# mitmul/chainer-faster-rcnn

Measured on AMD Instinct MI355X. Metric: images/sec VGG16 Faster R-CNN 600x1000, higher is better.
Workload: dtype f32; 1 GPU; VGG16 inference, 1xMI355X per image, batch 1, 300 proposals post-NMS, fp32 (BASELINE.json configs[1]); 1 image per GPU per step; image=1x3x600x1000, global_batch=1, launch=hipGraph replay, parallelism=dp1 (images sharded, no collective), n_rois_last_step=300

## Files before the change

chainer-faster-rcnn_amd/_lib.py:

```python
import ctypes
import os

HERE = os.path.dirname(os.path.abspath(__file__))
LIB_PATH = os.path.join(HERE, "libfrcnn_hip.so")

_P = ctypes.c_void_p
_I = ctypes.c_int
_D = ctypes.c_double
_F = ctypes.c_float
_S = ctypes.c_size_t

SIGNATURES = {
    "frcnn_abi_version": (_I, []),
    "frcnn_device_count": (_I, []),
    "frcnn_set_tuning": (_I, [ctypes.c_char_p, ctypes.c_char_p]),
    "frcnn_get_tuning": (_I, [ctypes.c_char_p, ctypes.c_char_p, _I]),
    "frcnn_reset_tuning": (_I, []),
    "frcnn_nms_workspace_bytes": (_S, [_I]),
    "frcnn_nms": (_I, [_P, _I, _D, _I, _P, _P, _P, _S, _P]),
    "frcnn_nms_batched_workspace_bytes": (_S, [_I, _I]),
    "frcnn_nms_batched": (_I, [_P, _I, _I, _D, _I, _P, _P, _P, _S, _P]),
    "frcnn_proposals_workspace_bytes": (_S, [_I, _I, _I, _I]),
    "frcnn_proposals": (_I, [_P, _P, _I, _I, _I, _P, _I, _I, _I, _F, _I, _I, _D, _P, _P, _P, _P, _P, _S, _P]),
    "frcnn_roi_pool_workspace_bytes": (_S, [_I, _I, _I]),
    "frcnn_chw_to_hwc": (_I, [_P, _I, _I, _I, _P, _P]),
    "frcnn_roi_pool_fwd_hwc": (_I, [_P, _I, _I, _I, _P, _I, _I, _I, _I, _F, _P, _P, _P]),
    "frcnn_roi_pool_fwd_chw": (_I, [_P, _I, _I, _I, _P, _I, _I, _I, _I, _F, _P, _P, _P, _S, _P]),
    "frcnn_roi_pool_fwd_chw_bf16": (_I, [_P, _I, _I, _I, _P, _I, _I, _I, _I, _F, _P, _P]),
    "frcnn_roi_pool_fwd_blk_bf16": (_I, [_P, _I, _I, _I, _P, _I, _I, _I, _I, _F, _P, _I, _P]),
    "frcnn_roi_pool_fwd_chw_f32s": (_I, [_P, _I, _I, _I, _P, _I, _I, _I, _I, _F, _P, _P]),
    "frcnn_roi_pool_fwd": (_I, [_P, _I, _I, _I, _P, _I, _I, _I, _F, _P, _P, _P, _S, _P]),
    "frcnn_roi_pool_bwd": (_I, [_P, _P, _I, _I, _I, _I, _I, _I, _P, _P]),
    "frcnn_roi_pool_bwd_ordered": (_I, [_P, _P, _I, _I, _I, _I, _I, _I, _P, _P]),
    "frcnn_pack_conv3x3_w": (_I, [_P, _I, _I, _P, _P]),
    "frcnn_conv3x3_workspace_bytes": (_S, [_I, _I, _I, _I]),
    "frcnn_conv3x3_workspace_init": (_I, [_P, _S, _P]),
    "frcnn_conv3x3_f32": (_I, [_P, _P, _P, _P, _I, _I, _I, _I, _I, _P, _S, _P]),
    "frcnn_conv3x3_f32_cfg": (_I, [_P, _P, _P, _P, _I, _I, _I, _I, _I, _I, _P, _S, _P]),
    "frcnn_wino_pack_w": (_I, [_P, _I, _I, _I, _P, _P]),
    "frcnn_conv_wino_workspace_bytes": (_S, [_I, _I, _I, _I]),
    "frcnn_conv3x3_wino_f32": (_I, [_P, _P, _P, _P, _I, _I, _I, _I, _I, _P, _S, _P]),
    "frcnn_maxpool2x2_f32": (_I, [_P, _P, _I, _I, _I, _P]),
    "frcnn_rpn_heads_padded_channels": (_I, [_I]),
    "frcnn_rpn_heads_pack": (_I, [_P, _P, _P, _P, _I, _I, _P, _P, _P]),
    "frcnn_rpn_heads_f32": (_I, [_P, _I, _I, _I, _I, _P, _P, _P, _P, _P]),
    "frcnn_linear_workspace_bytes": (_S, [_I, _I, _I]),
    "frcnn_linear_f32": (_I, [_P, _P, _P, _P, _I, _I, _I, _I, _P, _S, _P]),
    "frcnn_head_decode": (_I, [_P, _P, _P, _I, _I, _I, _I, _P, _P, _P]),
    "frcnn_head_decode_stacked": (_I, [_P, _P, _I, _I, _I, _I, _I, _I, _P, _P, _P]),
    "frcnn_preprocess_u8": (_I, [_P, _I, _I, _I, _P, _D, _I, _I, _P, _P]),
    "frcnn_class_dets": (_I, [_P, _P, _I, _I, _P, _P]),
    "frcnn_bbox_transform_inv": (_I, [_P, _P, _I, _I, _P, _P]),
    "frcnn_clip_boxes": (_I, [_P, _I, _I, _I, _P]),
    "frcnn_softmax_rows": (_I, [_P, _I, _I, _P, _P]),
    "frcnn_conv_f32_ex": (_I, [_P, _P, _P, _P, _P, _I, _I, _I, _I, _I, _I, _P, _S, _P]),
    "frcnn_f32s_pack_conv_w": (_I, [_P, _I, _I, _P, _P]),
    "frcnn_f32s_from_nchw_f32": (_I, [_P, _I, _I, _I, _P, _P]),
    "frcnn_f32s_to_nchw_f32": (_I, [_P, _I, _I, _I, _P, _P]),
    "frcnn_conv3x3_f32s": (_I, [_P, _P, _P, _P, _I, _I, _I, _I, _I, _I, _P]),
    "frcnn_conv1_f32s": (_I, [_P, _P, _P, _P, _I, _I, _I, _I, _I, _P]),
    "frcnn_conv1_bf16": (_I, [_P, _P, _P, _P, _I, _I, _I, _I, _I, _P]),
    "frcnn_conv1_f32": (_I, [_P, _P, _P, _P, _I, _I, _I, _I, _I, _P]),
    "frcnn_f32s_pack_from_packed": (_I, [_P, _I, _I, _I, _P, _P]),
    "frcnn_f32s_pack_many": (_I, [_P, _I, _P]),
    "frcnn_conv_wgrad_f32s": (_I, [_P, _P, _P, _I, _I, _I, _I, _P, _S, _P]),
    "frcnn_conv1_f32s_train": (_I, [_P, _P, _P, _P, _P, _I, _I, _I, _I, _I, _P]),
    "frcnn_conv3x3_f32s_train": (_I, [_P, _P, _P, _P, _P, _P, _I, _I, _I, _I, _I, _P, _S, _P]),
    "frcnn_bf16_pack_many": (_I, [_P, _I, _P]),
    "frcnn_conv1_bf16_train": (_I, [_P, _P, _P, _P, _P, _I, _I, _I, _I, _I, _P]),
    "frcnn_conv3x3_bf16_train": (_I, [_P, _P, _P, _P, _P, _P, _I, _I, _I, _I, _I, _P, _S, _P]),
    "frcnn_conv_wgrad_bf16_workspace_bytes": (_S, [_I, _I, _I, _I]),
    "frcnn_conv_wgrad_bf16": (_I, [_P, _P, _P, _I, _I, _I, _I, _P, _S, _P]),
    "frcnn_f16_pack_many": (_I, [_P, _I, _P]),
    "frcnn_conv1_f16_train": (_I, [_P, _P, _P, _P, _P, _I, _I, _I, _I, _I, _P]),
# ... 157 lines not shown
```

chainer-faster-rcnn_amd/csrc/conv_wino.hip:

```cpp
#include "frcnn_common.h"
#include <frcnn_buffer.h>
#include <frcnn_intrin.h>

typedef float f32x16 __attribute__((ext_vector_type(16)));

namespace {

constexpr int kWinoPitch = 40;
constexpr int kWinoLead = 3;

template <int CB, int TB, int CK, int BPC, bool SOFF>
__global__ void __launch_bounds__(256, BPC)
conv_wino_f32_kernel(const float *__restrict__ x, const float *__restrict__ u, const float *__restrict__ bias, float *__restrict__ y,
                     int Cin, int Cout, int H, int W, int mode, int xtiles, int ytiles, int nchunks, int piece_chunks) {
    constexpr int NT = 256;
    constexpr int BCO = 32 * CB;
    constexpr int HR = 4 * TB + 2;
    constexpr int WV = CK * 4 * BCO;
    constexpr int WIT = WV / NT;
    constexpr int HG = CK * HR * 10;
    constexpr int HIT4 = (HG + NT - 1) / NT;
    constexpr int HVP = (HG + 63) / 64 * 256;
    constexpr int WBUF = WV * 4;
    constexpr int ZF = 4 * 2 * TB * CB * 16 * 64;
    constexpr int MAINF = 2 * WBUF + 2 * HVP;
    constexpr int SMEM = MAINF > ZF ? MAINF : ZF;
    static_assert(WV % NT == 0, "U slab must split into whole per-thread float4s");
    static_assert(CK % 2 == 0 && CK * HR * 3 <= NT, "chunk shape");
    static_assert(SMEM * 4 <= 160 * 1024, "LDS");
    __shared__ __attribute__((aligned(16))) float smem[SMEM];

    const int tid = threadIdx.x, lane = tid & 63;
    const int wave = __builtin_amdgcn_readfirstlane(tid >> 6);
    const int l31 = lane & 31, khalf = lane >> 5;
    const int HW = H * W;
    const int npx = xtiles * ytiles, ntiles = npx * (Cout / BCO);
    int g = blockIdx.x;
    {
        const int G = gridDim.x, xcd = g & 7, q = G >> 3, r = G & 7;
        g = xcd * q + (xcd < r ? xcd : r) + (g >> 3);
    }
    const int piece = g / ntiles, tile = g % ntiles;
    const int pxt = tile % npx, cot = tile / npx;
    const int tx = pxt % xtiles, ty = pxt / xtiles;
    const int x0 = tx * 32, y0 = ty * 4 * TB, co0 = cot * BCO;
    const int c_begin = piece * piece_chunks;
    const int c_end = nchunks < c_begin + piece_chunks ? nchunks : c_begin + piece_chunks;
    const int K4 = Cin * 4;

    const frcnn_buf_t xbuf = frcnn_make_buf(x, (uint32_t)((size_t)Cin * HW * sizeof(float)));
    const frcnn_buf_t ubuf = frcnn_make_buf(u, (uint32_t)((size_t)K4 * Cout * 4 * sizeof(float)));
    const uint32_t u_chunk_bytes = (uint32_t)(CK * 4 * Cout * 4) * 4u, x_chunk_bytes = (uint32_t)(CK * HW) * 4u;

    uint32_t woff[WIT], hoff[HIT4];
#pragma unroll
    for (int q = 0; q < WIT; ++q) {
        const int v = tid + q * NT;
        const int row = v / BCO, c4 = v % BCO;
        woff[q] = (uint32_t)(row * Cout * 4 + (co0 + c4) * 4) * 4u;
    }
#pragma unroll
    for (int q = 0; q < HIT4; ++q) {
        const int e4 = tid + q * NT;
        const int c = e4 / (HR * 10), rem = e4 % (HR * 10);
        const int hr = rem / 10, g4 = rem % 10;
        const int gy = y0 - 1 + hr, gx = x0 - 4 + 4 * g4;
        const bool inside = e4 < HG && gy >= 0 && gy < H && gx >= 0 && gx < W;
        hoff[q] = inside ? (uint32_t)(c * HW + gy * W + gx) * 4u : kBufOob;
    }
    auto w_lds = [&](int buf) { return smem + buf * WBUF; };
    auto in_lds = [&](int buf) { return smem + 2 * WBUF + buf * HVP; };
    const int fix_lo = W - x0 + 4, fix_hi = (fix_lo + 3) & ~3;
    const bool edge_fix = (W & 3) != 0 && fix_lo > 0 && fix_lo < kWinoPitch;
    auto edge_zero = [&](int buf) {
        const int row = tid / 3, i = fix_lo + tid % 3;
        if (row < CK * HR && i < fix_hi) in_lds(buf)[row * kWinoPitch + i] = 0.0f;
        frcnn_barrier_nofence();
    };
    auto issue = [&](int chunk, int buf) {
        if constexpr (SOFF) {
            const uint32_t wb = (uint32_t)chunk * u_chunk_bytes, xb = (uint32_t)chunk * x_chunk_bytes;
#pragma unroll
            for (int q = 0; q < WIT; ++q) frcnn_buf_load_lds_b128(ubuf, w_lds(buf) + (q * NT + wave * 64) * 4, woff[q], wb);
#pragma unroll
            for (int q = 0; q < HIT4; ++q)
                if ((q + 1) * NT * 4 <= HVP || (wave * 64 + q * NT) * 4 < HVP)
                    frcnn_buf_load_lds_b128(xbuf, in_lds(buf) + (q * NT + wave * 64) * 4, hoff[q], xb);
        } else {
            const long long wrem = (long long)(K4 - chunk * CK * 4) * Cout * 4, xrem = (long long)(Cin - chunk * CK) * HW;
            const frcnn_buf_t ub_c = frcnn_make_buf(u + (size_t)chunk * CK * 4 * Cout * 4, (uint32_t)((wrem > 0 ? wrem : 0) * sizeof(float)));
            const frcnn_buf_t xb_c = frcnn_make_buf(x + (size_t)chunk * CK * HW, (uint32_t)((xrem > 0 ? xrem : 0) * sizeof(float)));
#pragma unroll
            for (int q = 0; q < WIT; ++q) frcnn_buf_load_lds_b128(ub_c, w_lds(buf) + (q * NT + wave * 64) * 4, woff[q], 0);
#pragma unroll
            for (int q = 0; q < HIT4; ++q)
                if ((q + 1) * NT * 4 <= HVP || (wave * 64 + q * NT) * 4 < HVP)
                    frcnn_buf_load_lds_b128(xb_c, in_lds(buf) + (q * NT + wave * 64) * 4, hoff[q], 0);
        }
    };

    f32x16 acc[TB][4][CB];
#pragma unroll
    for (int t = 0; t < TB; ++t)
#pragma unroll
        for (int k = 0; k < 4; ++k)
#pragma unroll
            for (int c = 0; c < CB; ++c)
#pragma unroll
                for (int r = 0; r < 16; ++r) acc[t][k][c][r] = 0.0f;

    const int ra = wave == 0 ? 0 : (wave == 2 ? 2 : 1);
    const int rb = wave == 0 ? 2 : (wave == 1 ? 2 : (wave == 2 ? 1 : 3));
    const float sb = wave == 1 ? 1.0f : -1.0f;
    const int tr = l31 >> 4, tc = l31 & 15;

    issue(c_begin, 0);
    frcnn_wait_vmcnt<0>();
    frcnn_barrier_nofence();
    if (edge_fix) edge_zero(0);
    int cur = 0;
    for (int chunk = c_begin; chunk < c_end; ++chunk) {
        const bool more = chunk + 1 < c_end;
        if (more) issue(chunk + 1, cur ^ 1);
        constexpr int NSTEP = CK / 2;
        const float *b_base = in_lds(cur) + (khalf * HR + 2 * tr) * kWinoPitch + kWinoLead + 2 * tc;
        const float *ba = b_base + ra * kWinoPitch, *bb = b_base + rb * kWinoPitch;
        const float4 *a_base = reinterpret_cast<const float4 *>(w_lds(cur)) + (khalf * 4 + wave) * BCO + l31;
        auto frag = [&](int s, float4 *a, float (*da)[4], float (*db)[4]) {
#pragma unroll
            for (int c = 0; c < CB; ++c) a[c] = a_base[2 * s * 4 * BCO + 32 * c];
#pragma unroll
            for (int t = 0; t < TB; ++t)
#pragma unroll
                for (int j = 0; j < 4; ++j) {
                    da[t][j] = ba[(2 * s * HR + 4 * t) * kWinoPitch + j];
                    db[t][j] = bb[(2 * s * HR + 4 * t) * kWinoPitch + j];
                }
        };
        float4 a[2][CB];
        float da[2][TB][4], db[2][TB][4];
        frag(0, a[0], da[0], db[0]);
#pragma unroll
        for (int s = 0; s < NSTEP; ++s) {
            if (s + 1 < NSTEP) frag(s + 1, a[(s + 1) & 1], da[(s + 1) & 1], db[(s + 1) & 1]);
            __builtin_amdgcn_sched_barrier(0);
#pragma unroll
            for (int t = 0; t < TB; ++t) {
                float tt[4];
#pragma unroll
                for (int j = 0; j < 4; ++j) tt[j] = fmaf(sb, db[s & 1][t][j], da[s & 1][t][j]);
                const float v[4] = {tt[0] - tt[2], tt[1] + tt[2], tt[2] - tt[1], tt[1] - tt[3]};
#pragma unroll
                for (int c = 0; c < CB; ++c) {
                    const float4 av = a[s & 1][c];
                    acc[t][0][c] = __builtin_amdgcn_mfma_f32_32x32x2f32(av.x, v[0], acc[t][0][c], 0, 0, 0);
                    acc[t][1][c] = __builtin_amdgcn_mfma_f32_32x32x2f32(av.y, v[1], acc[t][1][c], 0, 0, 0);
                    acc[t][2][c] = __builtin_amdgcn_mfma_f32_32x32x2f32(av.z, v[2], acc[t][2][c], 0, 0, 0);
                    acc[t][3][c] = __builtin_amdgcn_mfma_f32_32x32x2f32(av.w, v[3], acc[t][3][c], 0, 0, 0);
                }
            }
        }
        frcnn_wait_vmcnt<0>();
        frcnn_barrier_nofence();
        if (edge_fix && more) edge_zero(cur ^ 1);
        cur ^= 1;
    }

    float4 *z4 = reinterpret_cast<float4 *>(smem);
#pragma unroll
    for (int t = 0; t < TB; ++t)
#pragma unroll
        for (int c = 0; c < CB; ++c)
#pragma unroll
            for (int r4 = 0; r4 < 4; ++r4) {
                float z0[4], z1[4];
#pragma unroll
                for (int e = 0; e < 4; ++e) {
                    const int r = 4 * r4 + e;
                    z0[e] = (acc[t][0][c][r] + acc[t][1][c][r]) + acc[t][2][c][r];
                    z1[e] = (acc[t][1][c][r] - acc[t][2][c][r]) - acc[t][3][c][r];
                }
                z4[(((wave * 2 + 0) * TB * CB + t * CB + c) * 4 + r4) * 64 + lane] = make_float4(z0[0], z0[1], z0[2], z0[3]);
                z4[(((wave * 2 + 1) * TB * CB + t * CB + c) * 4 + r4) * 64 + lane] = make_float4(z1[0], z1[1], z1[2], z1[3]);
            }
    __syncthreads();
    const bool relu = (mode & 1) != 0, pool = (mode & 2) != 0, partial = (mode & 4) != 0;
    const int OH = (H + 1) / 2, OW = (W + 1) / 2;
#pragma unroll
    for (int t = 0; t < TB; ++t) {
        const int oy = y0 + 4 * t + 2 * tr, ox = x0 + 2 * tc;
        const bool in0 = oy < H && ox < W, has_r = ox + 1 < W, has_d = oy + 1 < H;
#pragma unroll
        for (int c = 0; c < CB; ++c) {
            float4 zz[4][2];
#pragma unroll
            for (int r = 0; r < 4; ++r)
#pragma unroll
                for (int q = 0; q < 2; ++q) zz[r][q] = z4[(((r * 2 + q) * TB * CB + t * CB + c) * 4 + wave) * 64 + lane];
            const int cob = co0 + 32 * c + 8 * wave + 4 * khalf;
            const float4 bq = partial ? make_float4(0.f, 0.f, 0.f, 0.f) : *reinterpret_cast<const float4 *>(&bias[cob]);
#pragma unroll
            for (int e = 0; e < 4; ++e) {
                auto comp = [&](const float4 &v) { return e == 0 ? v.x : (e == 1 ? v.y : (e == 2 ? v.z : v.w)); };
                float yv[2][2];
#pragma unroll
                for (int q = 0; q < 2; ++q) {
                    yv[0][q] = (comp(zz[0][q]) + comp(zz[1][q])) + comp(zz[2][q]);
                    yv[1][q] = (comp(zz[1][q]) - comp(zz[2][q])) - comp(zz[3][q]);
                }
                const float b = comp(bq);
                const int co = cob + e;
                if (!in0) continue;
                if (pool) {
                    float m = yv[0][0];
                    if (has_r) m = fmaxf(m, yv[0][1]);
                    if (has_d) m = fmaxf(m, yv[1][0]);
                    if (has_r && has_d) m = fmaxf(m, yv[1][1]);
                    y[(size_t)co * OH * OW + (size_t)(oy >> 1) * OW + (ox >> 1)] = fmaxf(m + b, 0.0f);
                } else {
                    float *yo = y + (partial ? (size_t)piece * Cout * HW : 0) + (size_t)co * HW + (size_t)oy * W + ox;
#pragma unroll
                    for (int p = 0; p < 2; ++p)
#pragma unroll
                        for (int q = 0; q < 2; ++q) {
                            if ((p && !has_d) || (q && !has_r)) continue;
                            float v = yv[p][q] + b;
                            if (relu) v = fmaxf(v, 0.0f);
                            yo[p * W + q] = v;
                        }
                }
            }
        }
    }
}

__global__ void __launch_bounds__(256)
wino_combine_kernel(const float *__restrict__ ws, const float *__restrict__ bias, float *__restrict__ y, int P, int C, int H, int W, int mode) {
    const size_t HW = (size_t)H * W, slab = (size_t)C * HW;
    const bool relu = (mode & 1) != 0, pool = (mode & 2) != 0;
    const int OH = pool ? (H + 1) / 2 : H, OW = pool ? (W + 1) / 2 : W;
    const size_t total = (size_t)C * OH * OW;
    for (size_t i = (size_t)blockIdx.x * blockDim.x + threadIdx.x; i < total; i += (size_t)gridDim.x * blockDim.x) {
        const int ow = (int)(i % OW), oh = (int)((i / OW) % OH), c = (int)(i / ((size_t)OW * OH));
        auto sum = [&](int yy, int xx) {
            const float *p = ws + (size_t)c * HW + (size_t)yy * W + xx;
            float s = p[0];
            for (int k = 1; k < P; ++k) s += p[(size_t)k * slab];
            return s;
        };
        if (pool) {
            const int yy = 2 * oh, xx = 2 * ow;
            float m = sum(yy, xx);
            if (xx + 1 < W) m = fmaxf(m, sum(yy, xx + 1));
            if (yy + 1 < H) m = fmaxf(m, sum(yy + 1, xx));
            if (xx + 1 < W && yy + 1 < H) m = fmaxf(m, sum(yy + 1, xx + 1));
            y[i] = fmaxf(m + bias[c], 0.0f);
        } else {
            float v = sum(oh, ow) + bias[c];
            y[i] = relu ? fmaxf(v, 0.0f) : v;
        }
    }
}

__global__ void __launch_bounds__(256)
wino_pack_w_kernel(const float *__restrict__ w, int Cout, int Cin, int packed, float *__restrict__ u) {
// ... 44 lines not shown
        hipLaunchKernelGGL(HIP_KERNEL_NAME(conv_wino_f32_kernel<CB, TB, CK, BPC, true>), dim3(G), dim3(256), 0, stream, x, u, bias, out, Cin, Cout, H, W,
                           kmode, p.xtiles, p.ytiles, p.nchunks, p.piece_chunks);
    else
        hipLaunchKernelGGL(HIP_KERNEL_NAME(conv_wino_f32_kernel<CB, TB, CK, BPC, false>), dim3(G), dim3(256), 0, stream, x, u, bias, out, Cin, Cout, H, W,
                           kmode, p.xtiles, p.ytiles, p.nchunks, p.piece_chunks);
    if (split) {
        const size_t total = (size_t)Cout * ((mode & 2) ? (size_t)((H + 1) / 2) * ((W + 1) / 2) : (size_t)H * W);
        const int blocks = (int)((total + 255) / 256 < 8192 ? (total + 255) / 256 : 8192);
        hipLaunchKernelGGL(wino_combine_kernel, dim3(blocks), dim3(256), 0, stream, (const float *)workspace, bias, y, p.pieces, Cout, H, W, mode);
    }
    return frcnn_launch_status();
}

static int pick_wino_config(int Cin, int Cout, int H, int W) {
    const int forced = frcnn_tune_int("FRCNN_CONV_WINO_CFG", 0);
    if (forced >= 1 && forced <= 2) return forced;
    (void)Cin; (void)Cout; (void)H; (void)W;
    return 1;
}

static int pick_wino_pieces(int cfg, int Cin, int Cout, int H, int W) {
    const int forced = frcnn_tune_int("FRCNN_CONV_WINO_SPLIT", 0);
    if (forced > 0) return forced;
    const int CK = cfg == 1 ? 8 : 4, BPC = 2;
    const long ntiles = (long)frcnn_cdiv(W, 32) * frcnn_cdiv(H, 4) * (Cout / 64);
    const long slots = (long)frcnn_cu_count() * BPC;
    const int nchunks = frcnn_cdiv(Cin, CK);
    if (ntiles >= 2 * slots) return 1;
    int pieces = (int)((2 * slots + ntiles - 1) / ntiles);
    const int maxp = nchunks / 4 > 1 ? nchunks / 4 : 1;
    return pieces < maxp ? pieces : maxp;
}

}

extern "C" {

int frcnn_wino_pack_w(const float *w, int Cout, int Cin, int packed, float *u, void *stream) {
    if (!w || !u || Cout < 1 || Cin < 1 || (packed != 0 && packed != 1)) return FRCNN_ERR_INVALID;
    hipLaunchKernelGGL(wino_pack_w_kernel, dim3(frcnn_cdiv(Cout * Cin, 256)), dim3(256), 0, (hipStream_t)stream, w, Cout, Cin, packed, u);
    return frcnn_launch_status();
}

size_t frcnn_conv_wino_workspace_bytes(int Cin, int Cout, int H, int W) {
    if (Cin < 1 || Cout < 1 || H < 1 || W < 1) return 0;
    size_t best = 256;
    for (int cfg = 1; cfg <= 2; ++cfg) {
        const int CK = cfg == 1 ? 8 : 4;
        int pieces = pick_wino_pieces(cfg, Cin, Cout, H, W);
        const int nchunks = frcnn_cdiv(Cin, CK);
        if (pieces > nchunks) pieces = nchunks;
        const int pc = frcnn_cdiv(nchunks, pieces > 0 ? pieces : 1);
        pieces = frcnn_cdiv(nchunks, pc);
        const size_t b = pieces > 1 ? frcnn_align256((size_t)pieces * Cout * H * W * sizeof(float)) : 256;
        if (b > best) best = b;
    }
    return best;
}

int frcnn_conv3x3_wino_f32(const float *x, const float *u, const float *bias, float *y, int Cin, int Cout, int H, int W, int act,
                           void *workspace, size_t workspace_bytes, void *stream_) {
    hipStream_t stream = (hipStream_t)stream_;
    if (!x || !u || !bias || !y || Cin < 1 || Cout < 1 || H < 1 || W < 1 || (Cout % 64) != 0) return FRCNN_ERR_INVALID;
    if (act != 0 && act != 1 && act != 4) return FRCNN_ERR_INVALID;
    if ((size_t)Cin * H * W * 4 >= (1ull << 31) || (size_t)Cin * 16 * Cout * 4 >= (1ull << 31)) return FRCNN_ERR_INVALID;
    const int mode = act == 4 ? 3 : act;
    const int cfg = pick_wino_config(Cin, Cout, H, W);
    const int pieces = pick_wino_pieces(cfg, Cin, Cout, H, W);
    switch (cfg) {
        case 2: return launch_wino<2, 1, 4, 2>(x, u, bias, y, Cin, Cout, H, W, mode, pieces, workspace, workspace_bytes, stream);
        default: return launch_wino<2, 1, 8, 2>(x, u, bias, y, Cin, Cout, H, W, mode, pieces, workspace, workspace_bytes, stream);
    }
}

}
```

chainer-faster-rcnn_amd/runtime.py:

```python
import ctypes

import numpy as np

from . import _lib
from . import tuning as _tuning

_NP = {"f32": np.float32, "i32": np.int32, "u8": np.uint8, "f64": np.float64, "i64": np.int64, "i16": np.int16}


class TorchDeviceMemory(object):

    def __init__(self, device="cuda:0"):
        import torch
        if not torch.cuda.is_available():
            raise _lib.FrcnnError("no HIP device visible to PyTorch: the MI355X path cannot run (no CPU fallback)")
        self.torch = torch
        self.device = torch.device(device)
        self._dt = {"f32": torch.float32, "i32": torch.int32, "u8": torch.uint8, "f64": torch.float64,
                    "i64": torch.int64, "i16": torch.int16}

    def empty(self, shape, dtype="f32"):
        return self.torch.empty(shape, dtype=self._dt[dtype], device=self.device)

    def zeros(self, shape, dtype="f32"):
# ... 403 lines not shown
                   "frcnn_bbox_transform_inv")
        return pred

    def clip_boxes_(self, boxes, im_h, im_w):
        m, L = self.mem, self.lib
        n = int(np.prod(boxes.shape)) // 4
        _lib.check(L.frcnn_clip_boxes(m.ptr(boxes), n, int(im_h), int(im_w), m.stream()), "frcnn_clip_boxes")
        return boxes

    def softmax_rows(self, scores):
        m, L = self.mem, self.lib
        R, n = int(scores.shape[0]), int(scores.shape[1])
        out = m.empty((R, n), "f32")
        _lib.check(L.frcnn_softmax_rows(m.ptr(scores), R, n, m.ptr(out), m.stream()), "frcnn_softmax_rows")
        return out


    def pack_wino_w(self, w, out=None):
        m, L = self.mem, self.lib
        packed = w.ndim == 2
        co, ci = (int(w.shape[1]), int(w.shape[0]) // 9) if packed else (int(w.shape[0]), int(w.shape[1]))
        u = out if out is not None else m.empty((ci * 16, co), "f32")
        assert tuple(u.shape) == (ci * 16, co)
        _lib.check(L.frcnn_wino_pack_w(m.ptr(w), co, ci, int(packed), m.ptr(u), m.stream()), "frcnn_wino_pack_w")
        return u

    def conv3x3_wino(self, x, u, bias, act=1, out=None):
        m, L = self.mem, self.lib
        ci, H, W = [int(v) for v in x.shape[-3:]]
        co = int(u.shape[1])
        assert int(u.shape[0]) == ci * 16
        oh, ow = ((H + 1) // 2, (W + 1) // 2) if act == 4 else (H, W)
        y = out if out is not None else m.empty((1, co, oh, ow), "f32")
        ws = self.workspace("conv_wino", L.frcnn_conv_wino_workspace_bytes(ci, co, H, W))
        _lib.check(L.frcnn_conv3x3_wino_f32(m.ptr(x), m.ptr(u), m.ptr(bias), m.ptr(y), ci, co, H, W, int(act), m.ptr(ws), ws.shape[0],
                                            m.stream()), "frcnn_conv3x3_wino_f32")
        return y

    def conv_ex(self, x, w_packed, bias, ksize=3, act=1, mask=None, out=None):
        m, L = self.mem, self.lib
        ci, H, W = [int(v) for v in x.shape[-3:]]
        co = int(w_packed.shape[1])
        assert int(w_packed.shape[0]) == ci * ksize * ksize
        oh, ow = ((H + 1) // 2, (W + 1) // 2) if act == 4 else (H, W)
        y = out if out is not None else m.empty((1, co, oh, ow), "f32")
        ws = self._conv_workspace(ci, co, H, W)
        _lib.check(L.frcnn_conv_f32_ex(m.ptr(x), m.ptr(w_packed), m.ptr(bias), m.ptr(mask), m.ptr(y), ci, co, H, W, int(ksize),
                                       int(act), m.ptr(ws), ws.shape[0], m.stream()), "frcnn_conv_f32_ex")
        return y

    def f32s_pack_conv_w(self, w):
        m, L = self.mem, self.lib
        co, ci = int(w.shape[0]), int(w.shape[1])
        wp = m.empty((3, self.bf16_pad(ci) // 16, 9, self.bf16_pad(co), 16), "i16")
        _lib.check(L.frcnn_f32s_pack_conv_w(m.ptr(w), co, ci, m.ptr(wp), m.stream()), "frcnn_f32s_pack_conv_w")
        return wp

    def f32s_from_nchw(self, x):
        m, L = self.mem, self.lib
        C, H, W = [int(v) for v in x.shape[-3:]]
        y = m.empty((3, self.bf16_pad(C) // 16, H, W, 16), "i16")
        _lib.check(L.frcnn_f32s_from_nchw_f32(m.ptr(x), C, H, W, m.ptr(y), m.stream()), "frcnn_f32s_from_nchw_f32")
        return y

    def f32s_to_nchw(self, x, C):
        m, L = self.mem, self.lib
# ... 571 lines not shown
```

include/frcnn_hip.h:

```cpp
#ifndef FRCNN_HIP_H
#define FRCNN_HIP_H
#include <stddef.h>
#include <stdint.h>

#ifdef __cplusplus
extern "C" {
#endif

#define FRCNN_OK 0
#define FRCNN_ERR_INVALID (-1)
#define FRCNN_ERR_UNSUPPORTED (-2)

int frcnn_abi_version(void);
int frcnn_device_count(void);

int frcnn_set_tuning(const char *key, const char *value);
int frcnn_get_tuning(const char *key, char *value_out, int capacity);
int frcnn_reset_tuning(void);

size_t frcnn_nms_workspace_bytes(int n);
int frcnn_nms(const float *dets, int n, double thresh, int max_out, int32_t *keep, int32_t *n_keep,
              void *workspace, size_t workspace_bytes, void *stream);

size_t frcnn_nms_batched_workspace_bytes(int groups, int n);
// ... 13 lines not shown
size_t frcnn_roi_pool_workspace_bytes(int C, int H, int W);
int frcnn_chw_to_hwc(const float *x, int C, int H, int W, float *xt, void *stream);
int frcnn_roi_pool_fwd_hwc(const float *xt, int C, int H, int W, const float *rois, int R, int roi_cols,
                           int outh, int outw, float spatial_scale, float *y, int32_t *argmax, void *stream);
int frcnn_roi_pool_fwd_chw(const float *x, int C, int H, int W, const float *rois, int R, int roi_cols,
                           int outh, int outw, float spatial_scale, float *y, int32_t *argmax, void *workspace,
                           size_t workspace_bytes, void *stream);
int frcnn_roi_pool_fwd_chw_f32s(const float *x, int C, int H, int W, const float *rois, int R, int roi_cols, int outh, int outw,
                                float spatial_scale, uint16_t *y_parts, void *stream);
int frcnn_roi_pool_fwd_chw_bf16(const float *x, int C, int H, int W, const float *rois, int R, int roi_cols, int outh,
                                int outw, float spatial_scale, uint16_t *y, void *stream);
int frcnn_roi_pool_fwd_blk_bf16(const uint16_t *x_blk, int C, int H, int W, const float *rois, int R, int roi_cols, int outh,
                                int outw, float spatial_scale, void *y, int out_bf16, void *stream);
int frcnn_roi_pool_fwd(const float *x, int C, int H, int W, const float *rois, int R, int outh, int outw,
                       float spatial_scale, float *y, int32_t *argmax, void *workspace,
                       size_t workspace_bytes, void *stream);
int frcnn_roi_pool_bwd(const float *dy, const int32_t *argmax, int R, int C, int H, int W, int outh,
                       int outw, float *dx, void *stream);

int frcnn_pack_conv3x3_w(const float *w, int Cout, int Cin, float *w_packed, void *stream);
size_t frcnn_conv3x3_workspace_bytes(int Cin, int Cout, int H, int W);
int frcnn_conv3x3_workspace_init(void *workspace, size_t workspace_bytes, void *stream);
int frcnn_conv3x3_f32(const float *x, const float *w_packed, const float *bias, float *y, int Cin,
                      int Cout, int H, int W, int relu, void *workspace, size_t workspace_bytes,
                      void *stream);
int frcnn_conv3x3_f32_cfg(const float *x, const float *w_packed, const float *bias, float *y, int Cin,
                          int Cout, int H, int W, int relu, int cfg, void *workspace,
                          size_t workspace_bytes, void *stream);
int frcnn_maxpool2x2_f32(const float *x, float *y, int C, int H, int W, void *stream);
int frcnn_wino_pack_w(const float *w, int Cout, int Cin, int packed, float *u, void *stream);
size_t frcnn_conv_wino_workspace_bytes(int Cin, int Cout, int H, int W);
int frcnn_conv3x3_wino_f32(const float *x, const float *u, const float *bias, float *y, int Cin, int Cout, int H, int W, int act,
                           void *workspace, size_t workspace_bytes, void *stream);

int frcnn_rpn_heads_padded_channels(int A);
int frcnn_rpn_heads_pack(const float *w_cls, const float *b_cls, const float *w_bbox, const float *b_bbox,
                         int Cmid, int A, float *w_packed, float *b_packed, void *stream);
int frcnn_rpn_heads_f32(const float *h, int Cmid, int H, int W, int A, const float *w_packed,
                        const float *b_packed, float *raw, float *cls_prob, void *stream);

size_t frcnn_linear_workspace_bytes(int M, int N, int K);
int frcnn_linear_f32(const float *x, const float *w, const float *bias, float *y, int M, int N, int K,
                     int relu, void *workspace, size_t workspace_bytes, void *stream);

int frcnn_head_decode(const float *boxes, const float *deltas, const float *cls_score, int R, int ncls,
                      int im_h, int im_w, float *pred_boxes, float *cls_prob, void *stream);
int frcnn_head_decode_stacked(const float *boxes, const float *out, int ld, int dcol, int R, int ncls, int im_h, int im_w,
                              float *pred_boxes, float *cls_prob, void *stream);
int frcnn_class_dets(const float *cls_prob, const float *pred_boxes, int R, int ncls, float *dets, void *stream);
int frcnn_preprocess_u8(const uint8_t *img, int H, int W, int C, const double *means_host, double im_scale, int OH, int OW,
                        float *out, void *stream);
int frcnn_bbox_transform_inv(const float *boxes, const float *deltas, int R, int ncls, float *pred_boxes,
                             void *stream);
int frcnn_clip_boxes(float *boxes, int n_boxes, int im_h, int im_w, void *stream);
int frcnn_softmax_rows(const float *scores, int R, int n, float *probs, void *stream);

int frcnn_conv_f32_ex(const float *x, const float *w_packed, const float *bias, const float *mask, float *y, int Cin,
                      int Cout, int H, int W, int ksize, int act, void *workspace, size_t workspace_bytes,
                      void *stream);

int frcnn_f32s_pack_conv_w(const float *w, int Cout, int Cin, uint16_t *w_packed, void *stream);
int frcnn_f32s_from_nchw_f32(const float *x, int C, int H, int W, uint16_t *y, void *stream);
int frcnn_f32s_to_nchw_f32(const uint16_t *x, int C, int H, int W, float *y, void *stream);
int frcnn_conv3x3_f32s(const uint16_t *x, const uint16_t *w_packed, const float *bias, void *y, int Cin, int Cout, int H,
                       int W, int relu, int out_mode, void *stream);
int frcnn_conv1_f32s(const float *x, const float *w, const float *bias, uint16_t *y, int Cin, int Cout, int H, int W, int relu,
// ... 205 lines not shown
```

Baseline: 380.1 img/s.

## Add stream-K Winograd conv kernel with in-kernel split-K fixup via tile counters

Result: faster. 393.1 img/s, median of 6 (+3.4%).

```diff
diff --git a/chainer-faster-rcnn_amd/_lib.py b/chainer-faster-rcnn_amd/_lib.py
--- a/chainer-faster-rcnn_amd/_lib.py
+++ b/chainer-faster-rcnn_amd/_lib.py
@@ -40,6 +40,9 @@
     "frcnn_wino_pack_w": (_I, [_P, _I, _I, _I, _P, _P]),
     "frcnn_conv_wino_workspace_bytes": (_S, [_I, _I, _I, _I]),
     "frcnn_conv3x3_wino_f32": (_I, [_P, _P, _P, _P, _I, _I, _I, _I, _I, _P, _S, _P]),
+    "frcnn_conv_wino_sk_workspace_bytes": (_S, [_I, _I, _I, _I]),
+    "frcnn_conv_wino_sk_workspace_init": (_I, [_P, _S, _P]),
+    "frcnn_conv3x3_wino_sk_f32": (_I, [_P, _P, _P, _P, _I, _I, _I, _I, _I, _P, _S, _P]),
     "frcnn_maxpool2x2_f32": (_I, [_P, _P, _I, _I, _I, _P]),
     "frcnn_rpn_heads_padded_channels": (_I, [_I]),
     "frcnn_rpn_heads_pack": (_I, [_P, _P, _P, _P, _I, _I, _P, _P, _P]),
diff --git a/chainer-faster-rcnn_amd/csrc/conv_wino.hip b/chainer-faster-rcnn_amd/csrc/conv_wino.hip
--- a/chainer-faster-rcnn_amd/csrc/conv_wino.hip
+++ b/chainer-faster-rcnn_amd/csrc/conv_wino.hip
@@ -1,4 +1,5 @@
 #include "frcnn_common.h"
+#include <frcnn_sync.h>
 #include <frcnn_buffer.h>
 #include <frcnn_intrin.h>
 
@@ -9,43 +10,34 @@
 constexpr int kWinoPitch = 40;
 constexpr int kWinoLead = 3;
 
-template <int CB, int TB, int CK, int BPC, bool SOFF>
-__global__ void __launch_bounds__(256, BPC)
-conv_wino_f32_kernel(const float *__restrict__ x, const float *__restrict__ u, const float *__restrict__ bias, float *__restrict__ y,
-                     int Cin, int Cout, int H, int W, int mode, int xtiles, int ytiles, int nchunks, int piece_chunks) {
-    constexpr int NT = 256;
-    constexpr int BCO = 32 * CB;
-    constexpr int HR = 4 * TB + 2;
-    constexpr int WV = CK * 4 * BCO;
-    constexpr int WIT = WV / NT;
-    constexpr int HG = CK * HR * 10;
-    constexpr int HIT4 = (HG + NT - 1) / NT;
-    constexpr int HVP = (HG + 63) / 64 * 256;
-    constexpr int WBUF = WV * 4;
-    constexpr int ZF = 4 * 2 * TB * CB * 16 * 64;
-    constexpr int MAINF = 2 * WBUF + 2 * HVP;
-    constexpr int SMEM = MAINF > ZF ? MAINF : ZF;
+template <int CB, int TB, int CK>
+struct WinoGeom {
+    static constexpr int NT = 256;
+    static constexpr int BCO = 32 * CB;
+    static constexpr int HR = 4 * TB + 2;
+    static constexpr int WV = CK * 4 * BCO;
+    static constexpr int WIT = WV / NT;
+    static constexpr int HG = CK * HR * 10;
+    static constexpr int HIT4 = (HG + NT - 1) / NT;
+    static constexpr int HVP = (HG + 63) / 64 * 256;
+    static constexpr int WBUF = WV * 4;
+    static constexpr int ZF = 4 * 2 * TB * CB * 16 * 64;
+    static constexpr int MAINF = 2 * WBUF + 2 * HVP;
+    static constexpr int SMEM = MAINF > ZF ? MAINF : ZF;
     static_assert(WV % NT == 0, "U slab must split into whole per-thread float4s");
     static_assert(CK % 2 == 0 && CK * HR * 3 <= NT, "chunk shape");
     static_assert(SMEM * 4 <= 160 * 1024, "LDS");
-    __shared__ __attribute__((aligned(16))) float smem[SMEM];
-
+};
+
+template <int CB, int TB, int CK, bool SOFF>
+__device__ __forceinline__ void wino_tile_loop(float *smem, const float *__restrict__ x, const float *__restrict__ u, int Cin, int Cout, int H, int W,
+                                               int x0, int y0, int co0, int c_begin, int c_end, f32x16 (&acc)[TB][4][CB]) {
+    using Geo = WinoGeom<CB, TB, CK>;
+    constexpr int NT = Geo::NT, BCO = Geo::BCO, HR = Geo::HR, WIT = Geo::WIT, HG = Geo::HG, HIT4 = Geo::HIT4, HVP = Geo::HVP, WBUF = Geo::WBUF;
     const int tid = threadIdx.x, lane = tid & 63;
     const int wave = __builtin_amdgcn_readfirstlane(tid >> 6);
     const int l31 = lane & 31, khalf = lane >> 5;
     const int HW = H * W;
-    const int npx = xtiles * ytiles, ntiles = npx * (Cout / BCO);
-    int g = blockIdx.x;
-    {
-        const int G = gridDim.x, xcd = g & 7, q = G >> 3, r = G & 7;
-        g = xcd * q + (xcd < r ? xcd : r) + (g >> 3);
-    }
-    const int piece = g / ntiles, tile = g % ntiles;
-    const int pxt = tile % npx, cot = tile / npx;
-    const int tx = pxt % xtiles, ty = pxt / xtiles;
-    const int x0 = tx * 32, y0 = ty * 4 * TB, co0 = cot * BCO;
-    const int c_begin = piece * piece_chunks;
-    const int c_end = nchunks < c_begin + piece_chunks ? nchunks : c_begin + piece_chunks;
     const int K4 = Cin * 4;
 
     const frcnn_buf_t xbuf = frcnn_make_buf(x, (uint32_t)((size_t)Cin * HW * sizeof(float)));
@@ -99,7 +91,6 @@
         }
     };
 
-    f32x16 acc[TB][4][CB];
 #pragma unroll
     for (int t = 0; t < TB; ++t)
 #pragma unroll
@@ -166,6 +157,12 @@
         cur ^= 1;
     }
 
+}
+
+template <int CB, int TB>
+__device__ __forceinline__ void wino_z_exchange(float *smem, const f32x16 (&acc)[TB][4][CB]) {
+    const int lane = threadIdx.x & 63;
+    const int wave = __builtin_amdgcn_readfirstlane(threadIdx.x >> 6);
     float4 *z4 = reinterpret_cast<float4 *>(smem);
 #pragma unroll
     for (int t = 0; t < TB; ++t)
@@ -184,53 +181,226 @@
                 z4[(((wave * 2 + 1) * TB * CB + t * CB + c) * 4 + r4) * 64 + lane] = make_float4(z1[0], z1[1], z1[2], z1[3]);
             }
     __syncthreads();
+}
+
+template <int CB, int TB>
+__device__ __forceinline__ void wino_y_of_z(const float *smem, int t, int c, float (&yv)[4][2][2]) {
+    const int lane = threadIdx.x & 63;
+    const int wave = __builtin_amdgcn_readfirstlane(threadIdx.x >> 6);
+    const float4 *z4 = reinterpret_cast<const float4 *>(smem);
+    float4 zz[4][2];
+#pragma unroll
+    for (int r = 0; r < 4; ++r)
+#pragma unroll
+        for (int q = 0; q < 2; ++q) zz[r][q] = z4[(((r * 2 + q) * TB * CB + t * CB + c) * 4 + wave) * 64 + lane];
+#pragma unroll
+    for (int e = 0; e < 4; ++e) {
+        auto comp = [&](const float4 &v) { return e == 0 ? v.x : (e == 1 ? v.y : (e == 2 ? v.z : v.w)); };
+#pragma unroll
+        for (int q = 0; q < 2; ++q) {
+            yv[e][0][q] = (comp(zz[0][q]) + comp(zz[1][q])) + comp(zz[2][q]);
+            yv[e][1][q] = (comp(zz[1][q]) - comp(zz[2][q])) - comp(zz[3][q]);
+        }
+    }
+}
+
+__device__ __forceinline__ void wino_emit(float *__restrict__ y, const float (&yv)[2][2], float b, int co, int oy, int ox, int H, int W, bool relu,
+                                          bool pool, bool has_r, bool has_d, size_t base) {
+    if (pool) {
+        const int OH = (H + 1) / 2, OW = (W + 1) / 2;
+        float m = yv[0][0];
+        if (has_r) m = fmaxf(m, yv[0][1]);
+        if (has_d) m = fmaxf(m, yv[1][0]);
+        if (has_r && has_d) m = fmaxf(m, yv[1][1]);
+        y[(size_t)co * OH * OW + (size_t)(oy >> 1) * OW + (ox >> 1)] = fmaxf(m + b, 0.0f);
+    } else {
+        float *yo = y + base + (size_t)co * H * W + (size_t)oy * W + ox;
+#pragma unroll
+        for (int p = 0; p < 2; ++p)
+#pragma unroll
+            for (int q = 0; q < 2; ++q) {
+                if ((p && !has_d) || (q && !has_r)) continue;
+                float v = yv[p][q] + b;
+                if (relu) v = fmaxf(v, 0.0f);
+                yo[p * W + q] = v;
+            }
+    }
+}
+
+template <int CB, int TB, int CK, int BPC, bool SOFF>
+__global__ void __launch_bounds__(256, BPC)
+conv_wino_f32_kernel(const float *__restrict__ x, const float *__restrict__ u, const float *__restrict__ bias, float *__restrict__ y,
+                     int Cin, int Cout, int H, int W, int mode, int xtiles, int ytiles, int nchunks, int piece_chunks) {
+    using Geo = WinoGeom<CB, TB, CK>;
+    constexpr int BCO = Geo::BCO;
+    __shared__ __attribute__((aligned(16))) float smem[Geo::SMEM];
+
+    const int tid = threadIdx.x, lane = tid & 63;
+    const int wave = __builtin_amdgcn_readfirstlane(tid >> 6);
+    const int l31 = lane & 31, khalf = lane >> 5;
+    const int HW = H * W;
+    const int npx = xtiles * ytiles, ntiles = npx * (Cout / BCO);
+    int g = blockIdx.x;
+    {
+        const int G = gridDim.x, xcd = g & 7, q = G >> 3, r = G & 7;
+        g = xcd * q + (xcd < r ? xcd : r) + (g >> 3);
+    }
+    const int piece = g / ntiles, tile = g % ntiles;
+    const int pxt = tile % npx, cot = tile / npx;
+    const int tx = pxt % xtiles, ty = pxt / xtiles;
+    const int x0 = tx * 32, y0 = ty * 4 * TB, co0 = cot * BCO;
+    const int c_begin = piece * piece_chunks;
+    const int c_end = nchunks < c_begin + piece_chunks ? nchunks : c_begin + piece_chunks;
+
+    f32x16 acc[TB][4][CB];
+    wino_tile_loop<CB, TB, CK, SOFF>(smem, x, u, Cin, Cout, H, W, x0, y0, co0, c_begin, c_end, acc);
+    wino_z_exchange<CB, TB>(smem, acc);
     const bool relu = (mode & 1) != 0, pool = (mode & 2) != 0, partial = (mode & 4) != 0;
-    const int OH = (H + 1) / 2, OW = (W + 1) / 2;
+    const int tr = l31 >> 4, tc = l31 & 15;
 #pragma unroll
     for (int t = 0; t < TB; ++t) {
         const int oy = y0 + 4 * t + 2 * tr, ox = x0 + 2 * tc;
         const bool in0 = oy < H && ox < W, has_r = ox + 1 < W, has_d = oy + 1 < H;
 #pragma unroll
         for (int c = 0; c < CB; ++c) {
-            float4 zz[4][2];
-#pragma unroll
-            for (int r = 0; r < 4; ++r)
-#pragma unroll
-                for (int q = 0; q < 2; ++q) zz[r][q] = z4[(((r * 2 + q) * TB * CB + t * CB + c) * 4 + wave) * 64 + lane];
+            float yv[4][2][2];
+            wino_y_of_z<CB, TB>(smem, t, c, yv);
             const int cob = co0 + 32 * c + 8 * wave + 4 * khalf;
             const float4 bq = partial ? make_float4(0.f, 0.f, 0.f, 0.f) : *reinterpret_cast<const float4 *>(&bias[cob]);
 #pragma unroll
             for (int e = 0; e < 4; ++e) {
-                auto comp = [&](const float4 &v) { return e == 0 ? v.x : (e == 1 ? v.y : (e == 2 ? v.z : v.w)); };
-                float yv[2][2];
-#pragma unroll
-                for (int q = 0; q < 2; ++q) {
-                    yv[0][q] = (comp(zz[0][q]) + comp(zz[1][q])) + comp(zz[2][q]);
-                    yv[1][q] = (comp(zz[1][q]) - comp(zz[2][q])) - comp(zz[3][q]);
+                const float b = e == 0 ? bq.x : (e == 1 ? bq.y : (e == 2 ? bq.z : bq.w));
+                if (!in0) continue;
+                wino_emit(y, yv[e], b, cob + e, oy, ox, H, W, relu, pool, has_r, has_d, partial ? (size_t)piece * Cout * HW : 0);
+            }
+        }
+    }
+}
+
+template <bool SOFF>
+__global__ void __launch_bounds__(256, 2)
+wino_sk_f32_kernel(const float *__restrict__ x, const float *__restrict__ u, const float *__restrict__ bias, float *__restrict__ y,
+                   int Cin, int Cout, int H, int W, int mode, int xtiles, int ytiles, int nchunks, long long total, int pieces, int piece_chunks,
+                   float *__restrict__ slots, int *__restrict__ tile_counters) {
+    constexpr int CB = 2, TB = 1, CK = 8;
+    using Geo = WinoGeom<CB, TB, CK>;
+    constexpr int BCO = Geo::BCO, NT = Geo::NT;
+    constexpr int SLOT_V = TB * CB * 4;
+    constexpr size_t kSlotFloats = (size_t)NT * SLOT_V * 4;
+    __shared__ __attribute__((aligned(16))) float smem[Geo::SMEM];
+
+    const int tid = threadIdx.x, lane = tid & 63;
+    const int wave = __builtin_amdgcn_readfirstlane(tid >> 6);
+    const int l31 = lane & 31, khalf = lane >> 5;
+    const int tr = l31 >> 4, tc = l31 & 15;
+    const int npx = xtiles * ytiles;
+    const long long G = gridDim.x;
+    long long g = blockIdx.x;
+    {
+        const long long xcd = g & 7, q = G >> 3, r = G & 7;
+        g = xcd * q + (xcd < r ? xcd : r) + (g >> 3);
+    }
+    auto start_of = [&](long long b) -> long long {
+        if (pieces > 0) {
+            const long long c = (b % pieces) * (long long)piece_chunks;
+            return (b / pieces) * nchunks + (c < nchunks ? c : nchunks);
+        }
+        return b * total / G;
+    };
+    auto owner_of = [&](long long i) -> long long {
+        if (pieces > 0) return (i / nchunks) * pieces + (i % nchunks) / piece_chunks;
+        long long b = i * G / total;
+        while (start_of(b + 1) <= i) ++b;
+        while (start_of(b) > i) --b;
+        return b;
+    };
+    const long long it_begin = start_of(g), it_end = start_of(g + 1);
+    const bool relu = (mode & 1) != 0, pool = (mode & 2) != 0;
+
+    for (long long it = it_begin; it < it_end;) {
+        const int tile = (int)(it / nchunks);
+        const int c_begin = (int)(it - (long long)tile * nchunks);
+        const int c_end = (int)((long long)nchunks < c_begin + (it_end - it) ? (long long)nchunks : c_begin + (it_end - it));
+        const int pxt = tile % npx, cot = tile / npx;
+        const int x0 = (pxt % xtiles) * 32, y0 = (pxt / xtiles) * 4 * TB, co0 = cot * BCO;
+        if (it != it_begin) __syncthreads();
+
+        f32x16 acc[TB][4][CB];
+        wino_tile_loop<CB, TB, CK, SOFF>(smem, x, u, Cin, Cout, H, W, x0, y0, co0, c_begin, c_end, acc);
+        wino_z_exchange<CB, TB>(smem, acc);
+
+        const bool whole = c_begin == 0 && c_end == nchunks;
+        float4 sum[SLOT_V];
+#pragma unroll
+        for (int t = 0; t < TB; ++t)
+#pragma unroll
+            for (int c = 0; c < CB; ++c) {
+                float yv[4][2][2];
+                wino_y_of_z<CB, TB>(smem, t, c, yv);
+#pragma unroll
+                for (int e = 0; e < 4; ++e) sum[(t * CB + c) * 4 + e] = make_float4(yv[e][0][0], yv[e][0][1], yv[e][1][0], yv[e][1][1]);
+            }
+        bool finish = true;
+        if (!whole) {
+            const long long t_first = (long long)tile * nchunks;
+            const long long g_first = owner_of(t_first), g_last = owner_of(t_first + nchunks - 1);
+            const int P = (int)(g_last - g_first + 1);
+            const int my_slot = (it == it_begin) ? 0 : 1;
+            const frcnn_buf_t pbuf = frcnn_make_buf(slots + ((size_t)g * 2 + my_slot) * kSlotFloats, (uint32_t)(kSlotFloats * sizeof(float)));
+#pragma unroll
+            for (int v = 0; v < SLOT_V; ++v)
+                frcnn_buf_store_f32x4_wt(pbuf, (uint32_t)((v * NT + tid) * 16),
+                                         make_float4(sum[v].x + 0.0f, sum[v].y + 0.0f, sum[v].z + 0.0f, sum[v].w + 0.0f));
+            frcnn_drain_vmem();
+            __syncthreads();
+            int *s_ticket = reinterpret_cast<int *>(smem);
+            if (tid == 0) *s_ticket = frcnn_ticket(&tile_counters[tile]);
+            __syncthreads();
+            finish = (*s_ticket == P - 1);
+            if (finish) {
+                if (tid == 0) {
+                    frcnn_acquire_agent();
+                    frcnn_counter_reset(&tile_counters[tile]);
                 }
-                const float b = comp(bq);
-                const int co = cob + e;
-                if (!in0) continue;
-                if (pool) {
-                    float m = yv[0][0];
-                    if (has_r) m = fmaxf(m, yv[0][1]);
-                    if (has_d) m = fmaxf(m, yv[1][0]);
-                    if (has_r && has_d) m = fmaxf(m, yv[1][1]);
-                    y[(size_t)co * OH * OW + (size_t)(oy >> 1) * OW + (ox >> 1)] = fmaxf(m + b, 0.0f);
-                } else {
-                    float *yo = y + (partial ? (size_t)piece * Cout * HW : 0) + (size_t)co * HW + (size_t)oy * W + ox;
-#pragma unroll
-                    for (int p = 0; p < 2; ++p)
-#pragma unroll
-                        for (int q = 0; q < 2; ++q) {
-                            if ((p && !has_d) || (q && !has_r)) continue;
-                            float v = yv[p][q] + b;
-                            if (relu) v = fmaxf(v, 0.0f);
-                            yo[p * W + q] = v;
-                        }
+                __syncthreads();
+                for (int q = 0; q < P; ++q) {
+                    const long long b = g_first + q;
+                    const int slot = (q == 0 && start_of(b) != t_first) ? 1 : 0;
+                    const float4 *piece = reinterpret_cast<const float4 *>(slots + ((size_t)b * 2 + slot) * kSlotFloats);
+                    float4 v[SLOT_V];
+#pragma unroll
+                    for (int e = 0; e < SLOT_V; ++e) v[e] = piece[(size_t)e * NT + tid];
+#pragma unroll
+                    for (int e = 0; e < SLOT_V; ++e) frcnn_pin(v[e]);
+#pragma unroll
+                    for (int e = 0; e < SLOT_V; ++e) {
+                        if (q == 0) sum[e] = v[e];
+                        else { sum[e].x += v[e].x; sum[e].y += v[e].y; sum[e].z += v[e].z; sum[e].w += v[e].w; }
+                    }
                 }
             }
         }
+        if (finish) {
+#pragma unroll
+            for (int t = 0; t < TB; ++t) {
+                const int oy = y0 + 4 * t + 2 * tr, ox = x0 + 2 * tc;
+                const bool in0 = oy < H && ox < W, has_r = ox + 1 < W, has_d = oy + 1 < H;
+#pragma unroll
+                for (int c = 0; c < CB; ++c) {
+                    const int cob = co0 + 32 * c + 8 * wave + 4 * khalf;
+                    const float4 bq = *reinterpret_cast<const float4 *>(&bias[cob]);
+#pragma unroll
+                    for (int e = 0; e < 4; ++e) {
+                        const float b = e == 0 ? bq.x : (e == 1 ? bq.y : (e == 2 ? bq.z : bq.w));
+                        const float4 sv = sum[(t * CB + c) * 4 + e];
+                        const float yv[2][2] = {{sv.x, sv.y}, {sv.z, sv.w}};
+                        if (!in0) continue;
+                        wino_emit(y, yv, b, cob + e, oy, ox, H, W, relu, pool, has_r, has_d, 0);
+                    }
+                }
+            }
+        }
+        it += c_end - c_begin;
     }
 }
 
@@ -341,6 +511,42 @@
     return pieces < maxp ? pieces : maxp;
 }
 
+
+constexpr size_t kWinoSkCounterPage = 64 * 1024;
+constexpr size_t kWinoSkSlotBytes = 64 * 4 * 32 * sizeof(float);
+
+struct WinoSkPlan { WinoPlan t; long long total; int G, pieces; bool classic, shared, self_cleaning; size_t counters_bytes, ws_bytes; };
+
+static WinoSkPlan plan_wino_sk(int Cin, int Cout, int H, int W) {
+    WinoSkPlan p;
+    const int forced_g = frcnn_tune_int("FRCNN_CONV_WINO_SK_G", 0);
+    int forced_p = frcnn_tune_int("FRCNN_CONV_WINO_SK_PIECES", 0);
+    const int classic_pieces = pick_wino_pieces(1, Cin, Cout, H, W);
+    if (forced_p < 0) forced_p = classic_pieces > 1 ? classic_pieces : 0;
+    const bool balance = frcnn_tune_int("FRCNN_CONV_WINO_SK_BALANCE", 0) == 1;
+    if (forced_p == 0 && forced_g <= 0 && !balance && classic_pieces > 1) forced_p = classic_pieces;
+    p.t = plan_wino<2, 1, 8>(Cin, Cout, H, W, forced_p > 0 ? forced_p : 1);
+    p.total = (long long)p.t.ntiles * p.t.nchunks;
+    p.classic = false;
+    p.pieces = 0;
+    if (forced_p > 0) {
+        p.pieces = p.t.pieces;
+        p.G = p.t.ntiles * p.t.pieces;
+        p.shared = p.t.pieces > 1;
+    } else {
+        const long long slots = 2LL * frcnn_cu_count();
+        if (forced_g > 0) p.G = (int)(forced_g < p.total ? forced_g : p.total);
+        else if (classic_pieces > 1) p.G = (int)(slots < p.total ? slots : p.total);
+        else { p.G = p.t.ntiles; p.classic = true; }
+        p.shared = p.G != p.t.ntiles;
+    }
+    const size_t need = frcnn_align256((size_t)p.t.ntiles * sizeof(int));
+    p.counters_bytes = need > kWinoSkCounterPage ? need : kWinoSkCounterPage;
+    p.self_cleaning = need <= kWinoSkCounterPage;
+    p.ws_bytes = p.shared ? p.counters_bytes + (size_t)p.G * 2 * kWinoSkSlotBytes : 0;
+    return p;
+}
+
 }
 
 extern "C" {
@@ -382,4 +588,38 @@
     }
 }
 
-}
+size_t frcnn_conv_wino_sk_workspace_bytes(int Cin, int Cout, int H, int W) {
+    if (Cin < 1 || Cout < 1 || H < 1 || W < 1 || (Cout % 64) != 0) return 0;
+    const WinoSkPlan p = plan_wino_sk(Cin, Cout, H, W);
+    return p.ws_bytes > kWinoSkCounterPage ? p.ws_bytes : kWinoSkCounterPage;
+}
+
+int frcnn_conv_wino_sk_workspace_init(void *workspace, size_t workspace_bytes, void *stream) {
+    if (!workspace || workspace_bytes < kWinoSkCounterPage) return FRCNN_ERR_INVALID;
+    FRCNN_HIP_TRY(hipMemsetAsync(workspace, 0, kWinoSkCounterPage, (hipStream_t)stream));
+    return FRCNN_OK;
+}
+
+int frcnn_conv3x3_wino_sk_f32(const float *x, const float *u, const float *bias, float *y, int Cin, int Cout, int H, int W, int act,
+                              void *workspace, size_t workspace_bytes, void *stream_) {
+    hipStream_t stream = (hipStream_t)stream_;
+    if (!x || !u || !bias || !y || Cin < 1 || Cout < 1 || H < 1 || W < 1 || (Cout % 64) != 0) return FRCNN_ERR_INVALID;
+    if (act != 0 && act != 1 && act != 4) return FRCNN_ERR_INVALID;
+    if ((size_t)Cin * H * W * 4 >= (1ull << 31) || (size_t)Cin * 16 * Cout * 4 >= (1ull << 31)) return FRCNN_ERR_INVALID;
+    const int mode = act == 4 ? 3 : act;
+    const WinoSkPlan p = plan_wino_sk(Cin, Cout, H, W);
+    if (p.classic) return launch_wino<2, 1, 8, 2>(x, u, bias, y, Cin, Cout, H, W, mode, 1, nullptr, 0, stream);
+    if (p.shared && (!workspace || workspace_bytes < p.ws_bytes)) return FRCNN_ERR_INVALID;
+    int *counters = p.shared ? (int *)workspace : nullptr;
+    float *slots = p.shared ? (float *)((char *)workspace + p.counters_bytes) : nullptr;
+    if (p.shared && !p.self_cleaning) FRCNN_HIP_TRY(hipMemsetAsync(counters, 0, p.counters_bytes, stream));
+    if (Cin % 8 == 0)
+        hipLaunchKernelGGL(HIP_KERNEL_NAME(wino_sk_f32_kernel<true>), dim3(p.G), dim3(256), 0, stream, x, u, bias, y, Cin, Cout, H, W, mode, p.t.xtiles,
+                           p.t.ytiles, p.t.nchunks, p.total, p.pieces, p.t.piece_chunks, slots, counters);
+    else
+        hipLaunchKernelGGL(HIP_KERNEL_NAME(wino_sk_f32_kernel<false>), dim3(p.G), dim3(256), 0, stream, x, u, bias, y, Cin, Cout, H, W, mode, p.t.xtiles,
+                           p.t.ytiles, p.t.nchunks, p.total, p.pieces, p.t.piece_chunks, slots, counters);
+    return frcnn_launch_status();
+}
+
+}
diff --git a/chainer-faster-rcnn_amd/runtime.py b/chainer-faster-rcnn_amd/runtime.py
--- a/chainer-faster-rcnn_amd/runtime.py
+++ b/chainer-faster-rcnn_amd/runtime.py
@@ -459,6 +459,14 @@
         assert int(u.shape[0]) == ci * 16
         oh, ow = ((H + 1) // 2, (W + 1) // 2) if act == 4 else (H, W)
         y = out if out is not None else m.empty((1, co, oh, ow), "f32")
+        classic = _tuning.get("FRCNN_CONV_WINO_SK", "1") == "0" or any(_tuning.get(k) is not None for k in ("FRCNN_CONV_WINO_CFG", "FRCNN_CONV_WINO_SPLIT"))
+        if not classic:
+            ws = self.workspace("conv_wino_sk", L.frcnn_conv_wino_sk_workspace_bytes(ci, co, H, W),
+                                init=lambda w: _lib.check(L.frcnn_conv_wino_sk_workspace_init(m.ptr(w), w.shape[0], m.stream()),
+                                                          "frcnn_conv_wino_sk_workspace_init"))
+            _lib.check(L.frcnn_conv3x3_wino_sk_f32(m.ptr(x), m.ptr(u), m.ptr(bias), m.ptr(y), ci, co, H, W, int(act), m.ptr(ws), ws.shape[0],
+                                                   m.stream()), "frcnn_conv3x3_wino_sk_f32")
+            return y
         ws = self.workspace("conv_wino", L.frcnn_conv_wino_workspace_bytes(ci, co, H, W))
         _lib.check(L.frcnn_conv3x3_wino_f32(m.ptr(x), m.ptr(u), m.ptr(bias), m.ptr(y), ci, co, H, W, int(act), m.ptr(ws), ws.shape[0],
                                             m.stream()), "frcnn_conv3x3_wino_f32")
diff --git a/include/frcnn_hip.h b/include/frcnn_hip.h
--- a/include/frcnn_hip.h
+++ b/include/frcnn_hip.h
@@ -69,6 +69,10 @@
 size_t frcnn_conv_wino_workspace_bytes(int Cin, int Cout, int H, int W);
 int frcnn_conv3x3_wino_f32(const float *x, const float *u, const float *bias, float *y, int Cin, int Cout, int H, int W, int act,
                            void *workspace, size_t workspace_bytes, void *stream);
+size_t frcnn_conv_wino_sk_workspace_bytes(int Cin, int Cout, int H, int W);
+int frcnn_conv_wino_sk_workspace_init(void *workspace, size_t workspace_bytes, void *stream);
+int frcnn_conv3x3_wino_sk_f32(const float *x, const float *u, const float *bias, float *y, int Cin, int Cout, int H, int W, int act,
+                              void *workspace, size_t workspace_bytes, void *stream);
 
 int frcnn_rpn_heads_padded_channels(int A);
 int frcnn_rpn_heads_pack(const float *w_cls, const float *b_cls, const float *w_bbox, const float *b_bbox,
```
